# vpc-ccg/tksm

Hardware: AMD Instinct MI355X
Metric: sequenced reads/s (higher is better)
Workload: dtype u8; 1 GPU; Bulk molecules, Badread error+qual model (nanopore2020, identity 84,99,5.5), 24 x 128 Mb random genome, FASTQ; kind=bulk, mean_len=1000, length_distribution=normal(1000, 200), compute_qual=True, contexts_in_flight_per_gpu=3

## Files before the change

__graft_entry__.py:

```python
import os
import subprocess
import sys

ROOT = os.path.dirname(os.path.abspath(__file__))


LLVM_BIN = "/opt/rocm/lib/llvm/bin"
NO_SPILL = ("k_alnf", "k_loop", "k_loopw", "k_err", "k_emit", "k_init")
LOOP_VGPR_LIMIT = 128
NO_SPILL_MDF = ("k_noise_plan", "k_noise_fill", "k_pal_count", "k_pal_write",
                "k_mut_count", "k_mut_write")
NO_SPILL_KDE = ("k_kde_grid", "k_kde_sum", "k_kde_cv_min", "k_kde_cv_sum")
NO_SPILL_ABUND = ("k_abund_compat", "k_abund_hits", "k_abund_msum", "k_abund_mfinish", "k_abund_mtotal", "k_abund_estep")
NO_SPILL_MS = ("k_ms_expand", "k_ms_err_events", "k_ms_qs_events")
NO_SPILL_BM = ("k_bm_match", "k_bm_adapter", "k_bm_exact")
NO_SPILL_MAP = ("k_map_chain", "k_map_sketch", "k_map_seed_write", "k_map_select")
NO_SPILL_MAP_ALIGN = ("k_map_align_path", "k_map_align", "k_map_align_encode")
NO_SPILL_MAP_EXTEND = ("k_map_extend", "k_map_extend_trace")


def kernel_resources(obj):
    import re
    import shutil
    import tempfile
# ... 23 lines not shown
                       ("map_kernels.o", NO_SPILL_MAP), ("map_align_kernels.o", NO_SPILL_MAP_ALIGN),
                       ("map_extend_kernels.o", NO_SPILL_MAP_EXTEND)):
        res = kernel_resources(os.path.join(ROOT, "tksm_amd", "csrc", "_build", obj))
        found = {n: r for n, r in res.items() if any(f"{len(k)}{k}" in n for k in names)}
        missing += [k for k in names if not any(f"{len(k)}{k}" in n for n in found)]
        guarded.update(found)
    if missing:
        raise RuntimeError(f"spill gate: kernels {missing} not found in the code object (renamed?)")
    bad = {n: r for n, r in guarded.items() if r.get("vgpr_spill_count", 0) or r.get("private_segment_fixed_size", 0)}
    if bad:
        raise RuntimeError("spill gate: scratch spills in " + "; ".join(
            f"{n}: {r.get('vgpr_spill_count')} VGPRs spilled, {r.get('private_segment_fixed_size')} B scratch" for n, r in bad.items()))
    return guarded


def build():
    subprocess.check_call(["make", "-s", "-j8", "-C", os.path.join(ROOT, "tksm_amd", "csrc")])
    guarded = check_no_spills()
    loop = [r for n, r in guarded.items() if "6k_loopE" in n]
    if len(loop) != 1 or loop[0]["vgpr_count"] > LOOP_VGPR_LIMIT:
        raise RuntimeError(f"k_loop: {[r['vgpr_count'] for r in loop]} VGPRs, the limit is {LOOP_VGPR_LIMIT}")
    print(f"k_loop: {loop[0]['vgpr_count']} VGPRs (limit {LOOP_VGPR_LIMIT}), no scratch; LDS per wave 256 B x fragment words per lane "
          f"(at most 64: 16 KB) + the 4 KB bounds table of the first thresholds")
    subprocess.check_call(["make", "-s", "-C", os.path.join(ROOT, "oracle")])
    sys.path.insert(0, ROOT)
    import tksm_amd
    from tksm_amd import _lib
    lib = _lib.load()
    missing = [s for s in _lib.SYMBOLS if not hasattr(lib, s)]
    if missing:
        raise RuntimeError(f"libtksmseq.so lacks symbols: {missing}")


def smoke():
    sys.path.insert(0, ROOT)
    sys.path.insert(0, os.path.join(ROOT, "oracle"))
    import numpy as np
    import pyoracle as po
    from tksm_amd.sequence import Sequencer
    models = os.path.join(ROOT, "tksm_amd", "models", "badread")
    err, qs = os.path.join(models, "nanopore2020.error.gz"), os.path.join(models, "nanopore2020.qscore.gz")
    rs = np.random.RandomState(3)
    ref = {f"c{i}": rs.choice(np.frombuffer(b"ACGT", np.uint8), 50_000).tobytes().decode() for i in range(2)}
    s = Sequencer(0)
    for k, v in ref.items():
        s.add_contig(k, v)
# ... 28 lines not shown
```

tksm_amd/csrc/ctx.h:

```cpp
#pragma once
#include <hip/hip_runtime.h>
#include <chrono>

#include <algorithm>
#include <cstdint>
#include <cstdio>
#include <cstdlib>
#include <map>
#include <memory>
#include <mutex>
#include <string>
#include <unordered_map>
#include <vector>

#include "../../include/tksmseq.h"
#include "abund_kernels.h"
#include "host.h"
#include "kernels.h"
#include "tsb_host.h"

using namespace tkh;

#define HIPCHK(ctx, call)                                                                         \
    do {                                                                                          \
// ... 244 lines not shown
    uint64_t total_bases = 0;
    uint32_t pool_blocks = 0;
    std::vector<uint8_t> contig_declared; uint32_t n_declared = 0;
    uint64_t ref_version = 0, wgs_version = ~0ull;
    DevBuf d_wgs_sofar, d_wgs_nameoff, d_wgs_namelen, d_wgs_names;
    DevBuf d_packed, d_blocktab, d_pool, d_contigs, d_stage;
    std::shared_ptr<const tsb::Transcripts> tsb;
    uint64_t tsb_dev_serial = 0, tsb_ref_version = ~0ull;
    DevBuf d_tsb_first, d_tsb_exons, d_tsb_lits, d_tsb_litpool;
    uint64_t tsb_n_lits = 0, tsb_lit_bytes = 0;
    float tsb_plan_ms = 0.f, tsb_write_ms = 0.f;
    uint64_t mut_serial = 0, mut_ref_version = ~0ull;
    DevBuf d_mut_refctg, d_mut_nameoff, d_mut_names, d_mut_delfirst, d_mut_ptfirst, d_mut_delfrom, d_mut_delto, d_mut_ptpos, d_mut_ptinfo, d_mut_insent, d_mut_inspool;

    ErrorModelHost em; QScoreModelHost qm; IdentityHost idm;
    bool em_uniform = false, em_alt0 = false;
    TailModelHost tail; uint64_t tail_version = 0;
    DevBuf d_tail_lx, d_tail_ly, d_tail_cdf, d_tail_chain;
    DevBuf d_pself, d_pseg, d_pt0, d_pt0b, d_cdf32, d_cdf, d_alts, d_altenc, d_nalts, d_qkeys, d_qoff, d_qcnt, d_qcdf, d_qq, d_qtab, d_qent, d_qpairs, d_qguide;

    DevBuf w_rawlen, w_slotcap, w_slotoff, w_outlen, w_ident, w_reclen, w_recoff, w_status, w_scan, w_trace, w_counter,
        w_scratch, w_records, w_istats, w_dstats, w_sums, w_fullpool, w_biglist, w_bigscratch, w_bigtrace;
    unsigned long long full_pool_bytes = 1ull << 30;
    DevBuf f_state, f_frag, f_nb, f_fplanes, f_jmeta[2], f_redo, f_jpopd, f_trace, f_tracefull, f_slow, f_defer, f_defercnt, f_frag2, f_row64;
    std::vector<uint32_t> h_row64;
    DevBuf f_round, f_geoall;
    PinnedBuf h_round, h_geo;
    bool force_slow = false;
    uint32_t tail_cut = 0;
    int tail_wcap = 2048;
    uint32_t tail_wave = 4096;
    uint32_t wave_loop = 16384;
    uint32_t full_rows_cap = 0;
    uint32_t small_aln = 131072;
    uint32_t n_buckets = 16;
    int defer_len = 0;
    int hbm_state_len = 2304;
    std::vector<hipEvent_t> evpool;
    uint32_t last_diag[DIAG_WORDS] = {};
    void* user_out = nullptr; uint64_t user_out_cap = 0;
    bool timing = false;
    int host_threads = 1;
    hipEvent_t ev[6] = {};
    tksmseq_result last{};
    bool have_last = false, have_stats = false;
    DevBuf g_counts, g_nlscan, g_sizes, g_offs, g_plans, g_out;
    tksmseq_gzip_result last_gzip{};
// ... 28 lines not shown
```

tksm_amd/csrc/kernels.h:

```cpp
#pragma once
#include <hip/hip_runtime.h>
#include <stdint.h>

namespace tk {

constexpr uint32_t NO_BLOCK = 0xFFFFFFFFu;
constexpr int BLOCK_SHIFT = 12;
constexpr int WAVES_PER_WG = 4;

struct RefView {
    const uint32_t* packed;
    const uint32_t* blocktab;
    const uint8_t* pool;
    const uint64_t* contigs;
    uint32_t n_contigs;
};

struct BatchView {
    const uint32_t* reads;
    const uint32_t* intervals;
    const uint32_t* mods;
    const uint64_t* literals;
    const uint8_t* litpool;
    const uint32_t* ids;
// ... 110 lines not shown
    CNT_SLOW = 2,
    CNT_FULL_ROWS = 3,
    CNT_EXIT = 4,
    CNT_REDO_JOBS = 8,
    CNT_REDO_WAVES = 9,
    CNT_REDO_LIST = 10,
    CNT_FAIL = 12,
    CNT_FAIL_OR = 13,
    CNT_FAIL_LAST = 14,
    CNT_FAIL_NM = 15,
    CNT_FAIL_REASON = 16,
    CNT_FAIL_QJOB = 24,
    CNT_FAIL_LIST = 25,
    CNT_EARLY_SLOW = 26,
    CNT_EARLY = 27,
    CNT_WORDS = 32
};
enum ExitCause { EXIT_BAND_LOOP = 0, EXIT_SHIFT_LOOP = 1, EXIT_SHIFT_ERR = 2, EXIT_BAND_ERR = 3 };
enum FailBit { FAIL_QUEUE = 0, FAIL_NOROW = 1, FAIL_SHIFT31 = 3, FAIL_SHIFT14 = 4, FAIL_END_CELL = 5, FAIL_WALK = 6 };

struct FastBuffers {
    ReadState* state;
    const uint32_t* row64;
    uint8_t* st_frag;
    uint16_t* st_nb;
    unsigned long long* st_fplanes;
    uint32_t* st_frag2;
    uint32_t* job_meta;
    uint8_t* job_popd;
    void* trace;
    uint32_t* redo_list;
    void* trace_full;
    uint32_t full_rows, full_tg;
    uint32_t full_cl;
    uint32_t* counters;
    uint32_t* job_cnt;
    uint32_t rs, n_ranges;
    const uint32_t* prev_meta; const uint8_t* prev_popd;
    const uint32_t* prefix;
    const uint32_t* base_cur; const uint32_t* base_prev;
    const RangeGeo* geo_cur; const RangeGeo* geo_prev;
    uint32_t* slow_list;
    uint32_t* early_hist;
    uint2* early_list;
    uint32_t* early_slow;
    uint2* defer_list;
    uint32_t* defer_cnt;
// ... 55 lines not shown
```

tksm_amd/csrc/kernels.hip:

```cpp
#include "kernels.h"
#include "loop_filter.h"
#include <type_traits>

namespace tk {

#define DEV __device__ __forceinline__

constexpr int BIG = 1 << 28;
DEV bool is_inf(int v) { return v >= (1 << 27); }

struct Ph4 { uint32_t x, y, z, w; };
enum { ST_ID = 0, ST_PAD = 1, ST_IDENT = 2, ST_DRAW = 3, ST_ALNPOS = 4, ST_QUAL = 5, ST_TAIL = 6 };

DEV Ph4 philox(uint64_t seed, uint64_t read, uint32_t stream, uint32_t n) {
    uint32_t c0 = (uint32_t)read, c1 = (uint32_t)(read >> 32), c2 = stream, c3 = n;
    uint32_t k0 = (uint32_t)seed, k1 = (uint32_t)(seed >> 32);
#pragma unroll
    for (int r = 0; r < 10; r++) {
        const unsigned long long p0 = (unsigned long long)0xD2511F53u * c0, p1 = (unsigned long long)0xCD9E8D57u * c2;
        const uint32_t h0 = (uint32_t)(p0 >> 32), l0 = (uint32_t)p0, h1 = (uint32_t)(p1 >> 32), l1 = (uint32_t)p1;
        uint32_t n0 = h1 ^ c1 ^ k0, n2 = h0 ^ c3 ^ k1;
        c0 = n0; c1 = l1; c2 = n2; c3 = l0;
        k0 += 0x9E3779B9u; k1 += 0xBB67AE85u;
    }
// ... 786 lines not shown
        }
    }
    if (a == 16) {
        uint4 v[4];
#pragma unroll
        for (int q = 0; q < 4; q++) v[q] = c4[4 + q];
#pragma unroll
        for (int q = 0; q < 4; q++) {
            a += !(w < v[q].x) ? 1 : 0; a += !(w < v[q].y) ? 1 : 0; a += !(w < v[q].z) ? 1 : 0; a += !(w < v[q].w) ? 1 : 0;
        }
    }
    return min(a, na);
}

DEV void go_slow(const FastBuffers& FB, uint64_t r, int lane, int cause) {
    if (lane == 0) {
        FB.state[r].slow = 1;
        atomicAdd(&FB.counters[CNT_EXIT + cause], 1u);
        const uint32_t idx = atomicAdd(&FB.counters[CNT_SLOW], 1u);
        FB.slow_list[idx] = (uint32_t)r;
    }
}

DEV uint8_t* frag_row(const FastBuffers& FB, uint64_t r) { return FB.st_frag + (size_t)FB.row64[r] * 64; }
DEV uint16_t* nb_row(const FastBuffers& FB, uint64_t r) { return FB.st_nb + (size_t)FB.row64[r] * 64; }
DEV unsigned long long* planes_row(const FastBuffers& FB, uint64_t r) { return FB.st_fplanes + 2 * ((size_t)FB.row64[r] + 8 * r); }
DEV int planes_words(const FastBuffers& FB, uint64_t r) { return (int)(FB.row64[r + 1] - FB.row64[r]) + 8; }
DEV uint32_t* frag2_row(const FastBuffers& FB, uint64_t r) { return FB.st_frag2 + 4 * ((size_t)FB.row64[r] + r); }
DEV int frag2_words(const FastBuffers& FB, uint64_t r) { return 4 * (int)(FB.row64[r + 1] - FB.row64[r]) + 4; }

DEV uint32_t early_bin(int L, double target) {
    const float sc = (float)L * (float)fmax(0.0, 1.0 - target);
    return (uint32_t)min(255, max(0, (int)(8.0f * __log2f(1.0f + sc))));
}
__global__ __launch_bounds__(256, 7) void k_init(BatchView B, RefView R, ErrModelView EM, IdentView IM, SimParams P,
                                               SimBuffers O, FastBuffers FB) {
#ifndef TKSM_ABLATE
    __builtin_amdgcn_s_setprio(2);
#endif
    const int lane = threadIdx.x & 63, wave = threadIdx.x >> 6, wpw = blockDim.x >> 6;
    const uint64_t r = (uint64_t)blockIdx.x * wpw + wave;
    if (r >= B.n_reads) return;
    uint8_t* frag = lds_raw + (size_t)wave * P.lcap;
    const int k = EM.k;
    const uint64_t g = P.first_read + r * P.stride;
    const int raw_len = (int)O.raw_len[r];
    const int L = raw_len + 2 * k;
    uint32_t status = 0;
    {
        const uint32_t ib = B.reads[2 * r], ic = B.reads[2 * r + 1];
        int o = k;
        for (uint32_t ii = 0; ii < ic; ii++) {
            const Ivl iv = load_interval(B, R, ib + ii);
            const int len = (int)iv.len;
            if (iv.literal) {
                const uint64_t lg = iv.gbase + iv.s;
                for (uint32_t t = (uint32_t)lane; t < (uint32_t)len; t += 64u) {
                    const uint8_t bch = upper(B.litpool[lg + (iv.minus ? (uint32_t)len - 1u - t : t)]);
                    frag[o + t] = iv.minus ? comp(bch) : bch;
                }
            } else
            for (uint32_t t0 = 16u * lane; t0 < (uint32_t)len; t0 += 1024u)
                splice_piece(B, R, iv.gbase + iv.s, (uint32_t)len, false, iv.minus, t0, frag + o + t0);
            wave_sync();
#pragma unroll 1
            for (uint32_t mi = iv.mod_begin; mi < iv.mod_end; mi++) {
// ... 2 lines not shown
                if (lane == 0) frag[o + (iv.minus ? len - 1 - (int)mp : (int)mp)] = iv.minus ? comp((uint8_t)mc) : (uint8_t)mc;
            }
            o += len;
        }
        if (O.tail_len && O.tail_len[r]) tail_fill(O.tail_chain, P.seed, g, frag + o, (int)O.tail_len[r], lane);
    }
    {
        const Ph4 pad = philox(P.seed, g, ST_PAD, 0);
        if (lane < k) {
            frag[lane] = base_char((int)(pad.x >> (2 * lane)));
            frag[k + raw_len + lane] = base_char((int)(pad.y >> (2 * lane)));
        }
    }
    double target;
    if (IM.constant) target = IM.value;
    else {
        const uint32_t u = philox(P.seed, g, ST_IDENT, 0).x;
        const uint32_t idx = u >> 16;
        const double fr = (double)(u & 0xffffu) * (1.0 / 65536.0);
        const double qa = IM.qtab[idx], qb = IM.qtab[idx + 1];
        target = IM.value * (qa + (qb - qa) * fr);
    }
    wave_sync();
    uint8_t* gfrag = frag_row(FB, r);
    unsigned long long* fpl = planes_row(FB, r);
    const int fw_r = planes_words(FB, r), fw2_r = frag2_words(FB, r);
    for (int t = 8 * lane; t < L; t += 512) {
        uint2 c = *reinterpret_cast<const uint2*>(frag + t);
        c.x = ((c.x >> 1) ^ (c.x >> 2)) & 0x03030303u; c.y = ((c.y >> 1) ^ (c.y >> 2)) & 0x03030303u;
        *reinterpret_cast<uint2*>(gfrag + t) = c;
    }
    {
        uint16_t* gnb0 = nb_row(FB, r);
        for (int t = 8 * lane; t < L; t += 512) {
            uint2 c = *reinterpret_cast<const uint2*>(frag + t);
            c.x = ((c.x >> 1) ^ (c.x >> 2)) & 0x03030303u; c.y = ((c.y >> 1) ^ (c.y >> 2)) & 0x03030303u;
            auto two = [](uint32_t b0, uint32_t b1) {
                return (0x1000u | (b0 & 1u) | ((b0 >> 1) << 5)) | ((0x1000u | (b1 & 1u) | ((b1 >> 1) << 5)) << 16);
            };
            uint4 o;
            o.x = two(c.x & 3u, (c.x >> 8) & 3u); o.y = two((c.x >> 16) & 3u, (c.x >> 24) & 3u);
            o.z = two(c.y & 3u, (c.y >> 8) & 3u); o.w = two((c.y >> 16) & 3u, (c.y >> 24) & 3u);
            if (t + 8 > L) {
                const int keep = L - t;
                uint32_t* ow = &o.x;
                for (int x2 = 0; x2 < 8; x2++) if (x2 >= keep) ow[x2 >> 1] &= (x2 & 1) ? 0x0000ffffu : 0xffff0000u;
            }
            *reinterpret_cast<uint4*>(gnb0 + t) = o;
        }
    }
    {
        uint32_t* f2 = frag2_row(FB, r);
        for (int w = lane; w < fw2_r; w += 64) {
            uint32_t word = 0u;
#pragma unroll
            for (int q = 0; q < 4; q++) {
                const int t = 16 * w + 4 * q;
                uint32_t c = t < P.lcap ? *reinterpret_cast<const uint32_t*>(frag + t) : 0u;
                if (t + 4 > L) c = t >= L ? 0u : c & (0xffffffffu >> (8 * (t + 4 - L)));
                const uint32_t codes4 = ((c >> 1) ^ (c >> 2)) & 0x03030303u;
                word |= ((codes4 * 0x40100401u) >> 24) << (24 - 8 * q);
            }
            f2[w] = word;
        }
    }
    bool dirty = false;
    const int nw = (L + 63) >> 6;
    for (int q0 = 0; q0 < fw_r; q0 += 64) {
        unsigned long long mylo = 0ull, myhi = 0ull;
        for (int q = q0; q < min(q0 + 64, nw); q++) {
            const int p = q * 64 + lane;
            const bool valid = p < L;
            const uint8_t c = valid ? frag[p] : (uint8_t)'A';
            const int code = code_of(c);
            dirty |= code < 0;
            const unsigned long long lo = __ballot(valid && (code & 1)), hi = __ballot(valid && (code & 2));
            if (lane == q - q0) { mylo = lo; myhi = hi; }
        }
        if (q0 + lane < fw_r) { ulonglong2 v; v.x = mylo; v.y = myhi; *reinterpret_cast<ulonglong2*>(fpl + 2 * (q0 + lane)) = v; }
    }
    const bool slow = __ballot(dirty) != 0ull;
    if (lane == 0) {
        ReadState S;
        S.errors = 0.0; S.target = target; S.est = 0.0; S.change_count = 0; S.n_base = 0; S.aln_no = 0;
        S.resume_src = -1; S.resume_j = 0; S.stage = 0; S.pending = 0; S.slow = slow ? 1 : 0; S.early = 0;
        S.st_draws = 0; S.st_aligns = 0; S.job = 0; S.raw_len = raw_len; S.res_mt = 0; S.res_cols = 0; S.res_fail = 0; S.pad3 = 0;
        FB.state[r] = S;
        O.status[r] |= status;
        if (slow) { const uint32_t idx = atomicAdd(&FB.counters[CNT_SLOW], 1u); FB.slow_list[idx] = (uint32_t)r; }
        else if (FB.early_hist) atomicAdd(&FB.early_hist[(blockIdx.x & 63u) * 256u + early_bin(L, target)], 1u);
    }
}

DEV void finish_read(const BatchView& B, const SimParams& P, const SimBuffers& O, uint64_t r, int raw_len, int out_len,
                     double identity, uint32_t status, int st_draws, int st_changes, int st_aligns, int L, int st_newlen,
                     int st_strim, int st_etrim, double errors, double target, int lane) {
    if (lane != 0) return;
    if (O.tail_len && !P.quirk_perfect) raw_len -= (int)O.tail_len[r];
    const long long h = pct_hundredths(identity);
    const uint32_t idl = B.ids[2 * r + 1];
    uint64_t rec = 1 + 36 + 8 + ndigits((unsigned)out_len) + 19 + ndigits((unsigned)raw_len) + 15 +
                   ndigits((unsigned long long)(h / 100)) + 3 + 14 + idl + 1;
// ... 43 lines not shown
        for (int jj = 0; jj < 8; jj++) {
            if (jj < k) {
                const uint32_t e = draw_slot(A, jj);
                if ((e >> 15) && (nb[i + jj] & 0x8000u) == 0) r.am |= 1u << jj;
                r.lens |= ((e >> 12) & 7u) << (3 * jj);
            }
        }
    }
    return r;
}

DEV int joined_len(const uint16_t* nb, int p0, int n, int lane) {
    int m = 0;
    for (int q = 0; q < n; q += 64) {
        const int p = q + lane;
        const int len = p < n ? slot_len(nb[p0 + p]) : 0;
        int total;
        (void)prefix_small(len, total);
        m += total;
    }
    return m;
}

DEV void join_out(const uint8_t* frag, const uint16_t* nb, int n, uint8_t* out_seq, int lo, int hi, int lane) {
    int base = 0;
    for (int q = 0; q < n; q += 64) {
        const int p = q + lane;
        uint32_t code = 0; int len = 0; uint8_t orig = 0;
        if (p < n) { code = nb[p]; len = slot_len(code); orig = frag[p]; }
        int total;
        const int off = base + prefix_small(len, total);
        const uint32_t syms = code ? code & 0x3ffu : planar1((uint32_t)orig);
        for (int x2 = 0; x2 < len; x2++) { const int c = off + x2; if (c >= lo && c < hi) out_seq[c - lo] = base_char((int)(((syms >> x2) & 1u) | (((syms >> (5 + x2)) & 1u) << 1))); }
        base += total;
    }
}

#ifndef TKSM_LOOP_N
#define TKSM_LOOP_N 16
#define TKSM_LOOP_K 3
#endif
constexpr int LOOP_N = TKSM_LOOP_N, LOOP_K = TKSM_LOOP_K;
__global__ __launch_bounds__(64) __attribute__((amdgpu_num_vgpr(128))) void k_loop(ErrModelView EM, SimParams P, FastBuffers FB, const uint32_t* __restrict__ order,
                                              uint32_t begin, uint32_t count, int Wl, int from_jobs, uint32_t c0, uint32_t c1) {
#ifndef TKSM_ABLATE
    __builtin_amdgcn_s_setprio(2);
#endif
    uint32_t* lf = reinterpret_cast<uint32_t*>(lds_raw);
    const int lane = threadIdx.x;
    const uint32_t widx = blockIdx.x * 64u + (uint32_t)lane;
    bool act = widx < count;
    uint32_t r = 0, rc = 0;
    if (act) {
        if (!from_jobs) { r = order[begin + widx]; rc = (begin + widx) / FB.rs; }
        else {
// ... 390 lines not shown
                sp->slow = 1;
                atomicAdd(&FB.counters[CNT_EXIT + EXIT_BAND_LOOP], 1u);
                FB.slow_list[atomicAdd(&FB.counters[CNT_SLOW], 1u)] = r;
            }
            return;
        }
        const uint32_t mt = S.res_mt, cols = S.res_cols;
        const double ident = cols ? (double)mt / (double)cols : 0.0;
        if (L <= 1000) errors = (1.0 - ident) * frag_len;
        else {
            const double estimated = (1.0 - ident) * frag_len;
            const double weight = 1000.0 / frag_len;
            errors = estimated * weight + errors * (1.0 - weight);
        }
        aln_no++;
    }
    const uint32_t kmer_range = (uint32_t)(L - k);
    const long long loop_limit = 100ll * L;
    const uint32_t kmask = (1u << (2 * k)) - 1u;
    int cc25 = change_count % 25;
    enum { RUN = 0, NEED_ALN = 1, DONE = 2 };
    int st = RUN;
    int st_aligns = S.st_aligns;
    const uint8_t* gfrag = frag_row(FB, r);
    if (TAIL && L <= 1000) { for (int t = lane; t < L; t += 64) Fw[t] = gfrag[t]; }
    for (;;) {
        while (st == RUN) {
            double est_cur = est_keep;
            if (resume_j == 0) {
                est_cur = 1.0 - div_inrange(errors, frag_len, rcp_len);
                if ((double)change_count > 0.9 * frag_len || est_cur <= target) { st = DONE; st_draws = (int)n; break; }
            }
            const uint32_t nl = n + (uint32_t)lane;
            const bool live = (long long)nl + 1 <= loop_limit;
            const Ph4 d = philox(P.seed, g, ST_DRAW, nl);
            const int di = (int)__umulhi(d.x, kmer_range);
            const int w = di >> 4, o = di & 15;
            const int kidx = (int)((uint32_t)(mk64(f2[w], f2[w + 1]) >> (64 - 2 * o - 2 * k)) & kmask);
            const uint4 seg = EM.pseg[kidx];
            const int na = EM.uniform_nalts ? EM.max_alts : (int)EM.nalts[kidx];
            int cls = EM.type == 0 ? 2 : (d.y < seg.x ? (EM.alt0_noop ? 0 : 3) : 1);
            const int sbase = 8 * ((d.y < seg.y ? 0 : 1) + (d.y < seg.z ? 0 : 1) + (d.y < seg.w ? 0 : 1));
            const uint4* c4 = reinterpret_cast<const uint4*>(EM.cdf32 + (cls == 1 ? (size_t)kidx * 32 + sbase : (size_t)0));
            const uint4 th0 = c4[0], th1 = c4[1];
            size_t at = 0;
            if (cls == 1 || cls == 3) {
                int a = 0;
                if (cls == 1) {
// ... 56 lines not shown
                wave_sync();
                if (stop_at >= 0) {
                    st = NEED_ALN;
                    if (stop_at + 1 < k) { resume_j = stop_at + 1; est_keep = est; n += (uint32_t)src; }
                    else { resume_j = 0; n += (uint32_t)src + 1u; }
                    break;
                }
                resume_j = 0;
                est_cur = 1.0 - div_inrange(errors, frag_len, rcp_len);
                if ((double)change_count > 0.9 * frag_len || est_cur <= target) { st = DONE; st_draws = (int)n + src + 1; break; }
            }
            if (st != RUN) break;
            resume_j = 0;
            if (dead) { st = DONE; st_draws = (int)loop_limit; break; }
            n += 64u;
        }
        if (!TAIL || st != NEED_ALN) break;
        {
            int p0 = 0, nrows = L;
            if (L > 1000) {
                p0 = (int)__umulhi(philox(P.seed, g, ST_ALNPOS, aln_no).x, (uint32_t)(L - 1000 + 1));
                nrows = 1000;
                wave_sync();
                for (int t = lane; t < nrows; t += 64) Fw[t] = gfrag[p0 + t];
            }
            wave_sync();
            const int m = join_window_planar(gnb, p0, nrows, Nw, ownw, wcap, lane);
            wave_sync();
            if (m > wcap) {
                if (early_mode) { to_exact_kernel(); return; }
                break;
            }
            const AlnOut a = band_align<0, false>(Fw, nrows, Nw, ownw, m, lane, nullptr);
            st_aligns++;
            if (is_inf(a.dist)) {
                to_exact_kernel();
                return;
            }
            const int cols = (int)(a.stat & 0xffffu), mt = (int)(a.stat >> 16);
            const double ident = cols ? (double)mt / (double)cols : 0.0;
            if (L <= 1000) errors = (1.0 - ident) * frag_len;
            else {
                const double estimated = (1.0 - ident) * frag_len;
                const double weight = 1000.0 / frag_len;
                errors = estimated * weight + errors * (1.0 - weight);
            }
            aln_no++;
// ... 32 lines not shown
    __builtin_amdgcn_s_setprio(2);
#endif
    const int lane = threadIdx.x & 63, wave = __builtin_amdgcn_readfirstlane(threadIdx.x >> 6), wpw = blockDim.x >> 6;
    const uint32_t widx = blockIdx.x * (uint32_t)wpw + (uint32_t)wave;
    if (widx >= count) return;
    uint64_t r; uint32_t pos;
    if (!from_jobs) { pos = begin + widx; r = (uint64_t)__builtin_amdgcn_readfirstlane((int)order[pos]) & 0xffffffffull; }
    else if (from_jobs == 2) {
        const uint2 e = FB.defer_list[widx];
        r = (uint64_t)__builtin_amdgcn_readfirstlane((int)e.x) & 0xffffffffull;
        pos = (uint32_t)__builtin_amdgcn_readfirstlane((int)e.y) * FB.rs;
    } else {
        const uint32_t target = FB.prefix[c0] + widx;
        uint32_t lo2 = c0, hi2 = c1 - 1;
        while (lo2 < hi2) { const uint32_t mid = (lo2 + hi2 + 1) >> 1; if (FB.prefix[mid] <= target) lo2 = mid; else hi2 = mid - 1; }
        const uint32_t pjob = FB.base_prev[lo2] + (target - FB.prefix[lo2]);
        r = (uint64_t)__builtin_amdgcn_readfirstlane((int)FB.prev_meta[4ull * pjob]) & 0xffffffffull;
        pos = lo2 * FB.rs;
    }
    ReadState S = FB.state[r];
    if (S.stage == 2 || S.slow) return;
    if (S.stage == 0) return;
    uint16_t* gnb = nb_row(FB, r);
    const int per_wave = STATE_IN_HBM ? lds_ncap + 128 : lds_lcap * 3 + lds_ncap + 128;
    uint8_t* lds_wave = lds_raw + (size_t)wave * per_wave;
    uint8_t* frag = STATE_IN_HBM ? frag_row(FB, r) : lds_wave;
    uint16_t* nb = STATE_IN_HBM ? gnb : reinterpret_cast<uint16_t*>(lds_wave + lds_lcap);
    uint8_t* aux = STATE_IN_HBM ? lds_wave : lds_wave + 3 * (size_t)lds_lcap;
    const int k = EM.k;
    const uint64_t g = P.first_read + r * P.stride;
    const int raw_len = __builtin_amdgcn_readfirstlane(S.raw_len);
    const int L = raw_len + 2 * k;
    const uint64_t slot = O.slot_off[r];
    const int cap = __builtin_amdgcn_readfirstlane((int)((O.slot_off[r + 1] - slot) >> 1));
    uint8_t* out_seq = O.scratch + slot;
    uint8_t* out_qual = out_seq + cap;
    if (!STATE_IN_HBM) {
        const uint8_t* gfrag0 = frag_row(FB, r);
        for (int t = lane * 4; t < L; t += 256) *reinterpret_cast<uint32_t*>(frag + t) = *reinterpret_cast<const uint32_t*>(gfrag0 + t);
        for (int t = lane * 2; t < L; t += 128) *reinterpret_cast<uint32_t*>(nb + t) = *reinterpret_cast<const uint32_t*>(gnb + t);
    }
    wave_sync();
    uint32_t status = 0;
    const double frag_len = (double)L;
    const double errors = S.errors;
    const double target = S.target;
    const int change_count = __builtin_amdgcn_readfirstlane(S.change_count), st_draws = __builtin_amdgcn_readfirstlane(S.st_draws);
    int st_aligns = __builtin_amdgcn_readfirstlane(S.st_aligns);
    double identity = 1.0;

    int start_trim, end_trim;
    {
        int v1 = lane < k ? slot_len(nb[lane]) : 0, v2 = lane < k ? slot_len(nb[L - k + lane]) : 0;
        (void)prefix_small(v1, start_trim);
        (void)prefix_small(v2, end_trim);
    }
    const int jcap = min(lds_ncap, cap);
    const int m = joined_len(nb, 0, L, lane);
    int lo = start_trim, hi = end_trim == 0 ? 0 : m - end_trim;
    lo = min(lo, m); hi = max(hi, lo);
    if (m > jcap) { status |= 1; lo = hi = 0; }
    const int out_len = hi - lo;
// ... 82 lines not shown
#ifdef TKSM_ABLATE
            if (P.ablate == 42) { out_qual[i2 - lo] = (uint8_t)(33 + (row & 31)); continue; }
            if (P.ablate == 43 && row >= 0) {
                const uint32_t w = (uint32_t)i2 * 2654435761u;
                const uint32_t a2 = QM.guide[(size_t)row * 64 + (w >> 26)] & 0x7fu;
                out_qual[i2 - lo] = (uint8_t)(33 + QM.pairs[roff + min(a2, rcnt - 1u)].y); continue;
            }
#endif
            if (row >= 0) {
                const uint32_t w = philox(P.seed, g, ST_QUAL, (uint32_t)i2).x;
                uint32_t a2 = QM.guide[(size_t)row * 64 + (w >> 26)];
                if (QM.guide_direct && (a2 & 0x80u)) q = (uint8_t)(a2 & 0x7fu);
                else {
                    uint2 pr = QM.pairs[roff + a2];
                    while (a2 + 1 < rcnt && !(w < pr.x)) { a2++; pr = QM.pairs[roff + a2]; }
                    q = (uint8_t)pr.y;
                }
            }
            out_qual[i2 - lo] = (uint8_t)(q + 33);
        }
    } else {
        identity = 1.0 - errors / frag_len;
    }
    join_out(frag, nb, L, out_seq, lo, hi, lane);
    if (P.quirk_perfect) identity = 1.0;
    finish_read(B, P, O, r, P.quirk_perfect ? out_len : raw_len, out_len, identity, status, st_draws, change_count, st_aligns, L, m,
                start_trim, end_trim, errors, target, lane);
    if (lane == 0) FB.state[r].stage = 2;
}

__global__ void k_collect_unfinished(FastBuffers FB, uint64_t n_reads) {
    const uint64_t r = (uint64_t)blockIdx.x * blockDim.x + threadIdx.x;
    if (r >= n_reads) return;
    ReadState S = FB.state[r];
    if (S.stage != 2 && !S.slow) {
        FB.state[r].slow = 1;
        const uint32_t idx = atomicAdd(&FB.counters[CNT_SLOW], 1u);
        FB.slow_list[idx] = (uint32_t)r;
    }
}

DEV uint32_t range_of_job(const FastBuffers& FB, uint32_t job0) {
    uint32_t rng = 0, hi2 = FB.n_ranges - 1;
    while (rng < hi2) { const uint32_t mid = (rng + hi2 + 1) >> 1; if (FB.base_cur[mid] <= job0) rng = mid; else hi2 = mid - 1; }
    return rng;
}
__global__ __launch_bounds__(64) void k_qjobs(FastBuffers FB, int k, uint32_t count) {
// ... 825 lines not shown
    if (per_cu > 8) per_cu = 8;
    if (per_cu < 1) per_cu = 1;
    return per_cu;
}
hipError_t launch_simulate(const BatchView& b, const RefView& r, const ErrModelView& em, const QsModelView& qm,
                           const IdentView& im, const SimParams& p, const SimBuffers& o, int n_wgs, int wpw, hipStream_t s) {
    if (!b.n_reads) return hipSuccess;
    const int lds = simulate_lds_bytes(p.s_lcap, p.s_ncap, wpw);
    hipError_t e = hipFuncSetAttribute(reinterpret_cast<const void*>(k_simulate<false>), hipFuncAttributeMaxDynamicSharedMemorySize, lds);
    if (e != hipSuccess) return e;
    hipLaunchKernelGGL(k_simulate<false>, dim3(n_wgs), dim3(64 * wpw), lds, s, b, r, em, qm, im, p, o);
    return hipGetLastError();
}
size_t simulate_big_bytes(int lcap, int ncap) { return ((size_t)lcap * 3 + (size_t)ncap * 6 + 255) & ~(size_t)255; }
hipError_t launch_simulate_big(const BatchView& b, const RefView& r, const ErrModelView& em, const QsModelView& qm,
                               const IdentView& im, const SimParams& p, const SimBuffers& o, int n_waves, hipStream_t s) {
    if (!b.n_reads || !n_waves) return hipSuccess;
    hipLaunchKernelGGL(k_simulate<true>, dim3(n_waves), dim3(64), 0, s, b, r, em, qm, im, p, o);
    return hipGetLastError();
}
hipError_t launch_init(const BatchView& b, const RefView& r, const ErrModelView& em, const IdentView& im, const SimParams& p,
                       const SimBuffers& o, const FastBuffers& fb, int wpw, hipStream_t s) {
    if (!b.n_reads) return hipSuccess;
    const int lds = wpw * p.lcap;
    hipError_t e = hipFuncSetAttribute(reinterpret_cast<const void*>(k_init), hipFuncAttributeMaxDynamicSharedMemorySize, lds);
    if (e != hipSuccess) return e;
    hipLaunchKernelGGL(k_init, dim3((unsigned)((b.n_reads + wpw - 1) / wpw)), dim3(64 * wpw), lds, s, b, r, em, im, p, o, fb);
    return hipGetLastError();
}
int err_lds_bytes(int lcap, int ncap, int wpw, bool state_in_hbm) { return wpw * ((state_in_hbm ? 0 : lcap * 3) + ncap + 128); }
hipError_t launch_err(const BatchView& b, const ErrModelView& em, const QsModelView& qm, const SimParams& p, const SimBuffers& o,
                      const FastBuffers& fb, const uint32_t* order, uint32_t begin, uint32_t count, int lds_lcap, int lds_ncap,
                      int from_jobs, uint32_t c0, uint32_t c1, int wpw, bool state_in_hbm, hipStream_t s) {
    if (!count) return hipSuccess;
    const int lds = err_lds_bytes(lds_lcap, lds_ncap, wpw, state_in_hbm);
    auto kern = state_in_hbm ? k_err<true> : k_err<false>;
    hipError_t e = hipFuncSetAttribute(reinterpret_cast<const void*>(kern), hipFuncAttributeMaxDynamicSharedMemorySize, 160 * 1024);
    if (e != hipSuccess) return e;
    hipLaunchKernelGGL(kern, dim3((count + wpw - 1) / wpw), dim3(64 * wpw), lds, s, b, em, qm, p, o, fb, order, begin, count, lds_lcap,
                       lds_ncap, from_jobs, c0, c1);
    return hipGetLastError();
}
constexpr int LOOP_WL_MAX = 64;
int loop_lds_words(int lcap) {
    static const int wl_max = [] { const char* e = getenv("TKSMSEQ_LOOP_WL"); return e ? std::max(4, atoi(e) & ~3) : LOOP_WL_MAX; }();
    return std::min(wl_max, (((lcap + 15) / 16 + 1) + 3) & ~3);
}
hipError_t launch_loop(const ErrModelView& em, const SimParams& p, const FastBuffers& fb, const uint32_t* order, uint32_t begin,
                       uint32_t count, int lcap, int from_jobs, uint32_t c0, uint32_t c1, hipStream_t s) {
    if (!count) return hipSuccess;
    const int Wl = loop_lds_words(lcap);
    hipLaunchKernelGGL(k_loop, dim3((count + 63) / 64), dim3(64), (size_t)Wl * 256 + tklf::LOOP_FILTER_BYTES, s, em, p, fb, order, begin, count, Wl, from_jobs, c0, c1);
    return hipGetLastError();
// ... 161 lines not shown
```

tksm_amd/csrc/run.cpp:

```cpp
#include "../../include/tksmseq.h"

#include <hip/hip_runtime.h>

#include <algorithm>
#include <cstdio>
#include <cstring>
#include <cstdlib>
#include <string>

#include "ctx.h"

#define TRY(call) do { const int rc_ = (call); if (rc_ != TKSMSEQ_OK) return rc_; } while (0)

static tk::BatchView batch_view(const tksmseq_batch* b) {
    return tk::BatchView{b->reads.as<uint32_t>(), b->intervals.as<uint32_t>(), b->mods.as<uint32_t>(), b->literals.as<uint64_t>(),
                         b->litpool.as<uint8_t>(), b->ids.as<uint32_t>(), b->idpool.as<uint8_t>(), b->n_reads, (uint32_t)b->n_literals};
}
static tk::RefView ref_view(const tksmseq_ctx* ctx) {
    return tk::RefView{ctx->d_packed.as<uint32_t>(), ctx->d_blocktab.as<uint32_t>(), ctx->d_pool.as<uint8_t>(),
                       ctx->d_contigs.as<uint64_t>(), (uint32_t)ctx->contig_names.size()};
}

static int apply_tail(tksmseq_ctx* ctx, tksmseq_batch* b, const tksmseq_run_params* p) {
    const bool want = p->mode == TKSMSEQ_MODE_BADREAD && ctx->tail.enabled && b->n_reads > 0;
// ... 174 lines not shown
        for (uint32_t c = 0; c < FB.n_ranges; c++) {
            r_ncap[c] = (uint32_t)pl.capf(b->raw_len[b->order[last_pos(c)]]);
            r_tg[c] = ((r_ncap[c] + 31) & ~31u) / 16 + 1;
            tot_trace += (uint64_t)FB.rs * r_tg[c]; tot_popd += (uint64_t)FB.rs * r_ncap[c];
        }
        ctx->h_row64.resize(n + 1);
        for (uint64_t r = 0; r < n; r++) { ctx->h_row64[r] = (uint32_t)nblk; nblk += ((uint64_t)b->raw_len[r] + 2 * pl.k + 63) / 64 + 1; }
        ctx->h_row64[n] = (uint32_t)nblk;
        nrb = (size_t)FB.n_ranges * 128;
        round_bytes = 2 * nrb + 1024;
        geo_off = (((size_t)(FB.n_ranges + 1) * 12 + 63) & ~(size_t)63);
        geo_bytes = geo_off + (size_t)FB.n_ranges * 2 * sizeof(tk::RangeGeo);
        FB.full_cl = ((((uint32_t)pl.ncap + 31) & ~31u) / 4 + 16 + 3) & ~3u;
        FB.full_tg = FB.full_cl + (FB.full_cl / 4 + 3) / 4 + 1;
        FB.full_rows = (uint32_t)std::max<uint64_t>(64, std::min<uint64_t>(jcap, (4ull << 30) / ((uint64_t)FB.full_tg * 64)) & ~63ull);
        full_rows_fit = FB.full_rows;
        if (ctx->full_rows_cap) FB.full_rows = std::min(FB.full_rows, std::max(64u, ctx->full_rows_cap & ~63u));
        early_on = ctx->early_tail > 0 && ctx->tail_cut == 0 && ctx->tail_wave > 0 && tk::tail_lds_bytes(pl.lcap) <= 65536 && n >= 16ull * ctx->early_tail;
    }
    int grow_buffers() {
        if (nblk >= (1ull << 32)) { ctx->err = "batch too large (split it)"; return TKSMSEQ_ELIMIT; }
        HIPCHK(ctx, ctx->f_state.ensure(n * sizeof(tk::ReadState) + 64));
        HIPCHK(ctx, ctx->f_row64.ensure((n + 1) * 4 + 64));
        HIPCHK(ctx, ctx->f_frag.ensure(nblk * 64 + 256));
        HIPCHK(ctx, ctx->f_nb.ensure(nblk * 128 + 256));
        HIPCHK(ctx, ctx->f_fplanes.ensure((nblk + 8 * n) * 16 + 256));
        HIPCHK(ctx, ctx->f_frag2.ensure((4 * nblk + 4 * n) * 4 + 1024));
        for (DevBuf& m : ctx->f_jmeta) HIPCHK(ctx, m.ensure(jcap * 16 + 64));
        HIPCHK(ctx, ctx->f_jpopd.ensure(tot_popd + 64));
        HIPCHK(ctx, ctx->f_round.ensure(round_bytes + 64));
        HIPCHK(ctx, ctx->f_geoall.ensure(geo_bytes + 64));
        HIPCHK(ctx, ctx->f_trace.ensure(tot_trace * 64 + 64));
        HIPCHK(ctx, ctx->f_redo.ensure(jcap * 4 + 64));
        HIPCHK(ctx, ctx->f_tracefull.ensure((size_t)FB.full_rows * FB.full_tg * 64 + 64));
        HIPCHK(ctx, ctx->f_slow.ensure(n * 4 + 64));
        HIPCHK(ctx, ctx->f_defer.ensure(n * 8 + 64));
        HIPCHK(ctx, ctx->f_defercnt.ensure((size_t)FB.n_ranges * 128 + 64));
        HIPCHK(ctx, ctx->h_round.ensure(round_bytes));
        HIPCHK(ctx, ctx->h_geo.ensure(geo_bytes));
        HIPCHK(ctx, hipMemcpyAsync(ctx->f_row64.p, ctx->h_row64.data(), (n + 1) * 4, hipMemcpyHostToDevice, s));
        FB.state = ctx->f_state.as<tk::ReadState>(); FB.st_frag = ctx->f_frag.as<uint8_t>(); FB.st_nb = ctx->f_nb.as<uint16_t>();
        FB.st_fplanes = ctx->f_fplanes.as<unsigned long long>(); FB.st_frag2 = ctx->f_frag2.as<uint32_t>(); FB.row64 = ctx->f_row64.as<uint32_t>();
        FB.trace = ctx->f_trace.p;
        FB.redo_list = ctx->f_redo.as<uint32_t>();
        FB.trace_full = ctx->f_tracefull.p; FB.counters = reinterpret_cast<uint32_t*>(ctx->f_round.as<uint8_t>() + nrb);
        FB.slow_list = ctx->f_slow.as<uint32_t>();
        FB.early_hist = nullptr; FB.early_list = nullptr; FB.early_slow = nullptr;
        if (early_on) {
            HIPCHK(ctx, ctx->f_early.ensure(65536 + (size_t)EARLY_CAP * 12 + 64));
            FB.early_hist = ctx->f_early.as<uint32_t>();
            FB.early_list = reinterpret_cast<uint2*>(ctx->f_early.as<uint8_t>() + 65536);
            FB.early_slow = reinterpret_cast<uint32_t*>(ctx->f_early.as<uint8_t>() + 65536 + (size_t)EARLY_CAP * 8);
            HIPCHK(ctx, hipMemsetAsync(ctx->f_early.p, 0, 65536, s));
        }
        FB.defer_list = ctx->f_defer.as<uint2>(); FB.defer_cnt = ctx->f_defercnt.as<uint32_t>(); FB.defer_len = ctx->defer_len;
        HIPCHK(ctx, hipMemsetAsync(ctx->f_defercnt.p, 0, (size_t)FB.n_ranges * 128, s));
        FB.prefix = ctx->f_geoall.as<uint32_t>(); FB.base_prev = FB.prefix + (FB.n_ranges + 1); FB.base_cur = FB.prefix + 2 * (FB.n_ranges + 1);
        FB.geo_cur = reinterpret_cast<tk::RangeGeo*>(ctx->f_geoall.as<uint8_t>() + geo_off); FB.geo_prev = FB.geo_cur + FB.n_ranges;
        return TKSMSEQ_OK;
    }
    void select_set(uint32_t round) {
        const int z = round & 1, y = z ^ 1;
        FB.job_meta = ctx->f_jmeta[z].as<uint32_t>(); FB.prev_meta = ctx->f_jmeta[y].as<uint32_t>();
        FB.prev_popd = FB.job_popd = ctx->f_jpopd.as<uint8_t>();
// ... 35 lines not shown
            Bucket bk;
            bk.begin = (uint32_t)i0; bk.count = (uint32_t)(i1 - i0);
            bk.lcap = (int)((mx + 2 * pl.k + 7) & ~7u); bk.ncap = (int)pl.capf(mx);
            bk.hbm = bk.lcap > ctx->hbm_state_len;
            bk.wpw = tk::WAVES_PER_WG;
            while (bk.wpw > 1 && tk::err_lds_bytes(bk.lcap, bk.ncap, bk.wpw, bk.hbm) > 64 * 1024) bk.wpw >>= 1;
            buckets.push_back(bk);
            i0 = i1;
        }
    }
    int prepare() {
        size_ranges();
        TRY(grow_buffers());
        select_set(0);
        HIPCHK(ctx, hipStreamSynchronize(s));
        memset(ctx->h_geo.p, 0, geo_bytes);
        const size_t nr1 = FB.n_ranges + 1;
        hprefix = ctx->h_geo.as<uint32_t>(); hbase_prev = hprefix + nr1; hbase_cur = hprefix + 2 * nr1;
        hrg = reinterpret_cast<tk::RangeGeo*>(ctx->h_geo.as<uint8_t>() + geo_off);
        for (uint32_t c = 0; c <= FB.n_ranges; c++) hbase_cur[c] = hbase_prev[c] = c * FB.rs;
        HIPCHK(ctx, place_ranges());
        cnt = ctx->h_round.as<uint32_t>() + nrb / 4;
        make_buckets();
        HIPCHK(ctx, hipMemsetAsync(ctx->f_nb.p, 0, nblk * 128, s));
        HIPCHK(ctx, hipMemsetAsync(ctx->f_round.p, 0, round_bytes, s));
        TRY(tick(GAP));
        pl.mark("buffers ready");
        return TKSMSEQ_OK;
    }
    int launch_side(uint32_t upto) {
        if (upto <= n_side || side_launches + 2 >= 1024) return TKSMSEQ_OK;
        const int k2 = (int)(side_launches % tksmseq_ctx::N_SIDE);
        HelperStream& h = ctx->side[k2];
        tk::SimBuffers O2 = pl.O;
        O2.read_list = ctx->f_slow.as<uint32_t>() + n_side; O2.n_work = upto - n_side;
        O2.work_counter = ctx->w_counter.as<unsigned long long>() + 1 + side_launches;
        O2.trace = pl.O.trace + ((size_t)pl.n_wgs * pl.wpw + (size_t)k2 * tksmseq_ctx::SIDE_WAVES) * pl.trace_words;
        HIPCHK(ctx, h.fork_from(s));
        const uint64_t want = (O2.n_work + pl.wpw - 1) / pl.wpw;
        const int wgs = (int)std::max<uint64_t>(1, std::min<uint64_t>(want, (uint64_t)(tksmseq_ctx::SIDE_WAVES / pl.wpw)));
        HIPCHK(ctx, tk::launch_simulate(pl.B, pl.R, pl.EM, pl.QM, pl.IM, pl.P, O2, wgs, pl.wpw, h.stream));
        HIPCHK(ctx, h.launched());
        n_side = upto; side_launches++;
        return TKSMSEQ_OK;
    }
    int launch_early(const std::vector<uint32_t>& copies) {
        uint32_t hist[256] = {};
// ... 325 lines not shown
```

Before: 15.39 million reads/s.

## Drop the byte fragment buffer and derive codes from packed planes

Removes the per-read byte-per-base fragment array from HBM. k_init now writes the 2-bit packed words, the nb slots and the bit planes in a single fused pass over LDS, with tail masking applied inline, so the separate memset of the nb buffer is no longer needed. The alignment window in k_loop rebuilds its codes from the frag2 words, and k_err reconstructs output bases from the nb slot codes alone, which frees one lcap of LDS per wave. The intent is less HBM traffic and memory footprint plus more LDS headroom, at the cost of extra unpacking arithmetic and a dependence on nb being fully initialised for every position.

```diff
diff --git a/__graft_entry__.py b/__graft_entry__.py
--- a/__graft_entry__.py
+++ b/__graft_entry__.py
@@ -69,6 +69,8 @@
         raise RuntimeError(f"k_loop: {[r['vgpr_count'] for r in loop]} VGPRs, the limit is {LOOP_VGPR_LIMIT}")
     print(f"k_loop: {loop[0]['vgpr_count']} VGPRs (limit {LOOP_VGPR_LIMIT}), no scratch; LDS per wave 256 B x fragment words per lane "
           f"(at most 64: 16 KB) + the 4 KB bounds table of the first thresholds")
+    for kern, tag in (("k_init", "6k_initE"), ("k_err<false>", "5k_errILb0EE"), ("k_err<true>", "5k_errILb1EE")):
+        print(f"{kern}: " + ", ".join(f"{r['vgpr_count']} VGPRs, no scratch" for n, r in guarded.items() if tag in n))
     subprocess.check_call(["make", "-s", "-C", os.path.join(ROOT, "oracle")])
     sys.path.insert(0, ROOT)
     import tksm_amd
diff --git a/tksm_amd/csrc/ctx.h b/tksm_amd/csrc/ctx.h
--- a/tksm_amd/csrc/ctx.h
+++ b/tksm_amd/csrc/ctx.h
@@ -290,7 +290,7 @@
     DevBuf w_rawlen, w_slotcap, w_slotoff, w_outlen, w_ident, w_reclen, w_recoff, w_status, w_scan, w_trace, w_counter,
         w_scratch, w_records, w_istats, w_dstats, w_sums, w_fullpool, w_biglist, w_bigscratch, w_bigtrace;
     unsigned long long full_pool_bytes = 1ull << 30;
-    DevBuf f_state, f_frag, f_nb, f_fplanes, f_jmeta[2], f_redo, f_jpopd, f_trace, f_tracefull, f_slow, f_defer, f_defercnt, f_frag2, f_row64;
+    DevBuf f_state, f_nb, f_fplanes, f_jmeta[2], f_redo, f_jpopd, f_trace, f_tracefull, f_slow, f_defer, f_defercnt, f_frag2, f_row64;
     std::vector<uint32_t> h_row64;
     DevBuf f_round, f_geoall;
     PinnedBuf h_round, h_geo;
diff --git a/tksm_amd/csrc/kernels.h b/tksm_amd/csrc/kernels.h
--- a/tksm_amd/csrc/kernels.h
+++ b/tksm_amd/csrc/kernels.h
@@ -156,7 +156,6 @@
 struct FastBuffers {
     ReadState* state;
     const uint32_t* row64;
-    uint8_t* st_frag;
     uint16_t* st_nb;
     unsigned long long* st_fplanes;
     uint32_t* st_frag2;
diff --git a/tksm_amd/csrc/kernels.hip b/tksm_amd/csrc/kernels.hip
--- a/tksm_amd/csrc/kernels.hip
+++ b/tksm_amd/csrc/kernels.hip
@@ -832,7 +832,6 @@
     }
 }
 
-DEV uint8_t* frag_row(const FastBuffers& FB, uint64_t r) { return FB.st_frag + (size_t)FB.row64[r] * 64; }
 DEV uint16_t* nb_row(const FastBuffers& FB, uint64_t r) { return FB.st_nb + (size_t)FB.row64[r] * 64; }
 DEV unsigned long long* planes_row(const FastBuffers& FB, uint64_t r) { return FB.st_fplanes + 2 * ((size_t)FB.row64[r] + 8 * r); }
 DEV int planes_words(const FastBuffers& FB, uint64_t r) { return (int)(FB.row64[r + 1] - FB.row64[r]) + 8; }
@@ -843,6 +842,7 @@
     const float sc = (float)L * (float)fmax(0.0, 1.0 - target);
     return (uint32_t)min(255, max(0, (int)(8.0f * __log2f(1.0f + sc))));
 }
+__host__ __device__ inline int init_lds_stride(int lcap) { return (lcap + 15) & ~15; }
 __global__ __launch_bounds__(256, 7) void k_init(BatchView B, RefView R, ErrModelView EM, IdentView IM, SimParams P,
                                                SimBuffers O, FastBuffers FB) {
 #ifndef TKSM_ABLATE
@@ -851,7 +851,7 @@
     const int lane = threadIdx.x & 63, wave = threadIdx.x >> 6, wpw = blockDim.x >> 6;
     const uint64_t r = (uint64_t)blockIdx.x * wpw + wave;
     if (r >= B.n_reads) return;
-    uint8_t* frag = lds_raw + (size_t)wave * P.lcap;
+    uint8_t* frag = lds_raw + (size_t)wave * init_lds_stride(P.lcap);
     const int k = EM.k;
     const uint64_t g = P.first_read + r * P.stride;
     const int raw_len = (int)O.raw_len[r];
@@ -900,62 +900,48 @@
         target = IM.value * (qa + (qb - qa) * fr);
     }
     wave_sync();
-    uint8_t* gfrag = frag_row(FB, r);
     unsigned long long* fpl = planes_row(FB, r);
-    const int fw_r = planes_words(FB, r), fw2_r = frag2_words(FB, r);
-    for (int t = 8 * lane; t < L; t += 512) {
-        uint2 c = *reinterpret_cast<const uint2*>(frag + t);
-        c.x = ((c.x >> 1) ^ (c.x >> 2)) & 0x03030303u; c.y = ((c.y >> 1) ^ (c.y >> 2)) & 0x03030303u;
-        *reinterpret_cast<uint2*>(gfrag + t) = c;
-    }
-    {
-        uint16_t* gnb0 = nb_row(FB, r);
-        for (int t = 8 * lane; t < L; t += 512) {
-            uint2 c = *reinterpret_cast<const uint2*>(frag + t);
-            c.x = ((c.x >> 1) ^ (c.x >> 2)) & 0x03030303u; c.y = ((c.y >> 1) ^ (c.y >> 2)) & 0x03030303u;
-            auto two = [](uint32_t b0, uint32_t b1) {
-                return (0x1000u | (b0 & 1u) | ((b0 >> 1) << 5)) | ((0x1000u | (b1 & 1u) | ((b1 >> 1) << 5)) << 16);
-            };
-            uint4 o;
-            o.x = two(c.x & 3u, (c.x >> 8) & 3u); o.y = two((c.x >> 16) & 3u, (c.x >> 24) & 3u);
-            o.z = two(c.y & 3u, (c.y >> 8) & 3u); o.w = two((c.y >> 16) & 3u, (c.y >> 24) & 3u);
-            if (t + 8 > L) {
-                const int keep = L - t;
-                uint32_t* ow = &o.x;
-                for (int x2 = 0; x2 < 8; x2++) if (x2 >= keep) ow[x2 >> 1] &= (x2 & 1) ? 0x0000ffffu : 0xffff0000u;
-            }
-            *reinterpret_cast<uint4*>(gnb0 + t) = o;
-        }
-    }
-    {
-        uint32_t* f2 = frag2_row(FB, r);
-        for (int w = lane; w < fw2_r; w += 64) {
-            uint32_t word = 0u;
-#pragma unroll
-            for (int q = 0; q < 4; q++) {
-                const int t = 16 * w + 4 * q;
-                uint32_t c = t < P.lcap ? *reinterpret_cast<const uint32_t*>(frag + t) : 0u;
-                if (t + 4 > L) c = t >= L ? 0u : c & (0xffffffffu >> (8 * (t + 4 - L)));
-                const uint32_t codes4 = ((c >> 1) ^ (c >> 2)) & 0x03030303u;
-                word |= ((codes4 * 0x40100401u) >> 24) << (24 - 8 * q);
-            }
-            f2[w] = word;
-        }
-    }
+    uint16_t* gnb0 = nb_row(FB, r);
+    uint32_t* f2 = frag2_row(FB, r);
+    const int nb64 = (int)(FB.row64[r + 1] - FB.row64[r]);
+    const int fw_r = nb64 + 8, fw2_r = 4 * nb64 + 4;
     bool dirty = false;
-    const int nw = (L + 63) >> 6;
-    for (int q0 = 0; q0 < fw_r; q0 += 64) {
-        unsigned long long mylo = 0ull, myhi = 0ull;
-        for (int q = q0; q < min(q0 + 64, nw); q++) {
-            const int p = q * 64 + lane;
-            const bool valid = p < L;
-            const uint8_t c = valid ? frag[p] : (uint8_t)'A';
-            const int code = code_of(c);
-            dirty |= code < 0;
-            const unsigned long long lo = __ballot(valid && (code & 1)), hi = __ballot(valid && (code & 2));
-            if (lane == q - q0) { mylo = lo; myhi = hi; }
-        }
-        if (q0 + lane < fw_r) { ulonglong2 v; v.x = mylo; v.y = myhi; *reinterpret_cast<ulonglong2*>(fpl + 2 * (q0 + lane)) = v; }
+    for (int w0 = 0; w0 < 4 * fw_r; w0 += 64) {
+        const int w = w0 + lane, t = 16 * w, nv = L - t;
+        uint4 c = make_uint4(0u, 0u, 0u, 0u);
+        if (nv > 0) c = *reinterpret_cast<const uint4*>(frag + t);
+        const uint32_t c4[4] = {c.x, c.y, c.z, c.w};
+        uint32_t word = 0u, lo16 = 0u, hi16 = 0u, sc[8];
+#pragma unroll
+        for (int q = 0; q < 4; q++) {
+            const int nq = nv - 4 * q;
+            const uint32_t vm = nq >= 4 ? 0xffffffffu : nq <= 0 ? 0u : (1u << (8 * nq)) - 1u;
+            const uint32_t cd = ((c4[q] >> 1) ^ (c4[q] >> 2)) & 0x03030303u & vm;
+            const uint32_t b0 = cd & 0x01010101u, b1 = (cd >> 1) & 0x01010101u;
+            dirty |= ((c4[q] ^ (0x41414141u + 2u * b0 + 6u * b1 + 11u * (b0 & b1))) & vm) != 0u;
+            word |= ((cd * 0x40100401u) >> 24) << (24 - 8 * q);
+            lo16 |= ((b0 * 0x01020408u) >> 24) << (4 * q);
+            hi16 |= ((b1 * 0x01020408u) >> 24) << (4 * q);
+            const uint32_t cv = cd | (vm & 0x04040404u);
+            const uint32_t y0 = __builtin_amdgcn_perm(cv, cv, 0x0c010c00u), y1 = __builtin_amdgcn_perm(cv, cv, 0x0c030c02u);
+            sc[2 * q] = (y0 & 0x00010001u) | ((y0 & 0x00020002u) << 4) | ((y0 & 0x00040004u) << 10);
+            sc[2 * q + 1] = (y1 & 0x00010001u) | ((y1 & 0x00020002u) << 4) | ((y1 & 0x00040004u) << 10);
+        }
+        if (w < fw2_r) f2[w] = word;
+        if (w < 4 * nb64) {
+            uint4* d = reinterpret_cast<uint4*>(gnb0 + t);
+            d[0] = make_uint4(sc[0], sc[1], sc[2], sc[3]);
+            d[1] = make_uint4(sc[4], sc[5], sc[6], sc[7]);
+        }
+        const int pc = (int)(lo16 | (hi16 << 16));
+        const uint32_t p0 = (uint32_t)dpp_mov<0x00, 0xf>(0, pc), p1 = (uint32_t)dpp_mov<0x55, 0xf>(0, pc),
+                       p2 = (uint32_t)dpp_mov<0xaa, 0xf>(0, pc), p3 = (uint32_t)dpp_mov<0xff, 0xf>(0, pc);
+        if ((lane & 3) == 0 && (w >> 2) < fw_r) {
+            ulonglong2 v;
+            v.x = mk64((p2 & 0xffffu) | (p3 << 16), (p0 & 0xffffu) | (p1 << 16));
+            v.y = mk64((p2 >> 16) | (p3 & 0xffff0000u), (p0 >> 16) | (p1 & 0xffff0000u));
+            *reinterpret_cast<ulonglong2*>(fpl + 2 * (w >> 2)) = v;
+        }
     }
     const bool slow = __ballot(dirty) != 0ull;
     if (lane == 0) {
@@ -1045,15 +1031,15 @@
     return m;
 }
 
-DEV void join_out(const uint8_t* frag, const uint16_t* nb, int n, uint8_t* out_seq, int lo, int hi, int lane) {
+DEV void join_out(const uint16_t* nb, int n, uint8_t* out_seq, int lo, int hi, int lane) {
     int base = 0;
     for (int q = 0; q < n; q += 64) {
         const int p = q + lane;
-        uint32_t code = 0; int len = 0; uint8_t orig = 0;
-        if (p < n) { code = nb[p]; len = slot_len(code); orig = frag[p]; }
+        uint32_t code = 0; int len = 0;
+        if (p < n) { code = nb[p]; len = slot_len(code); }
         int total;
         const int off = base + prefix_small(len, total);
-        const uint32_t syms = code ? code & 0x3ffu : planar1((uint32_t)orig);
+        const uint32_t syms = code & 0x3ffu;
         for (int x2 = 0; x2 < len; x2++) { const int c = off + x2; if (c >= lo && c < hi) out_seq[c - lo] = base_char((int)(((syms >> x2) & 1u) | (((syms >> (5 + x2)) & 1u) << 1))); }
         base += total;
     }
@@ -1490,8 +1476,17 @@
     enum { RUN = 0, NEED_ALN = 1, DONE = 2 };
     int st = RUN;
     int st_aligns = S.st_aligns;
-    const uint8_t* gfrag = frag_row(FB, r);
-    if (TAIL && L <= 1000) { for (int t = lane; t < L; t += 64) Fw[t] = gfrag[t]; }
+    auto window_codes = [&](int p0, int nrows) {
+        for (int t = 16 * lane; t < nrows; t += 1024) {
+            const int x = p0 + t, w = x >> 4, o = x & 15;
+            const uint32_t c16 = (uint32_t)((mk64(f2[w], f2[w + 1]) << (2 * o)) >> 32);
+            uint32_t b[4] = {0u, 0u, 0u, 0u};
+#pragma unroll
+            for (int j = 0; j < 16; j++) b[j >> 2] |= ((c16 >> (30 - 2 * j)) & 3u) << (8 * (j & 3));
+            *reinterpret_cast<uint4*>(Fw + t) = make_uint4(b[0], b[1], b[2], b[3]);
+        }
+    };
+    if (TAIL && L <= 1000) window_codes(0, L);
     for (;;) {
         while (st == RUN) {
             double est_cur = est_keep;
@@ -1594,7 +1589,7 @@
                 p0 = (int)__umulhi(philox(P.seed, g, ST_ALNPOS, aln_no).x, (uint32_t)(L - 1000 + 1));
                 nrows = 1000;
                 wave_sync();
-                for (int t = lane; t < nrows; t += 64) Fw[t] = gfrag[p0 + t];
+                window_codes(p0, nrows);
             }
             wave_sync();
             const int m = join_window_planar(gnb, p0, nrows, Nw, ownw, wcap, lane);
@@ -1673,11 +1668,10 @@
     if (S.stage == 2 || S.slow) return;
     if (S.stage == 0) return;
     uint16_t* gnb = nb_row(FB, r);
-    const int per_wave = STATE_IN_HBM ? lds_ncap + 128 : lds_lcap * 3 + lds_ncap + 128;
+    const int per_wave = STATE_IN_HBM ? lds_ncap + 128 : lds_lcap * 2 + lds_ncap + 128;
     uint8_t* lds_wave = lds_raw + (size_t)wave * per_wave;
-    uint8_t* frag = STATE_IN_HBM ? frag_row(FB, r) : lds_wave;
-    uint16_t* nb = STATE_IN_HBM ? gnb : reinterpret_cast<uint16_t*>(lds_wave + lds_lcap);
-    uint8_t* aux = STATE_IN_HBM ? lds_wave : lds_wave + 3 * (size_t)lds_lcap;
+    uint16_t* nb = STATE_IN_HBM ? gnb : reinterpret_cast<uint16_t*>(lds_wave);
+    uint8_t* aux = STATE_IN_HBM ? lds_wave : lds_wave + 2 * (size_t)lds_lcap;
     const int k = EM.k;
     const uint64_t g = P.first_read + r * P.stride;
     const int raw_len = __builtin_amdgcn_readfirstlane(S.raw_len);
@@ -1687,8 +1681,6 @@
     uint8_t* out_seq = O.scratch + slot;
     uint8_t* out_qual = out_seq + cap;
     if (!STATE_IN_HBM) {
-        const uint8_t* gfrag0 = frag_row(FB, r);
-        for (int t = lane * 4; t < L; t += 256) *reinterpret_cast<uint32_t*>(frag + t) = *reinterpret_cast<const uint32_t*>(gfrag0 + t);
         for (int t = lane * 2; t < L; t += 128) *reinterpret_cast<uint32_t*>(nb + t) = *reinterpret_cast<const uint32_t*>(gnb + t);
     }
     wave_sync();
@@ -1817,7 +1809,7 @@
     } else {
         identity = 1.0 - errors / frag_len;
     }
-    join_out(frag, nb, L, out_seq, lo, hi, lane);
+    join_out(nb, L, out_seq, lo, hi, lane);
     if (P.quirk_perfect) identity = 1.0;
     finish_read(B, P, O, r, P.quirk_perfect ? out_len : raw_len, out_len, identity, status, st_draws, change_count, st_aligns, L, m,
                 start_trim, end_trim, errors, target, lane);
@@ -2689,13 +2681,13 @@
 hipError_t launch_init(const BatchView& b, const RefView& r, const ErrModelView& em, const IdentView& im, const SimParams& p,
                        const SimBuffers& o, const FastBuffers& fb, int wpw, hipStream_t s) {
     if (!b.n_reads) return hipSuccess;
-    const int lds = wpw * p.lcap;
+    const int lds = wpw * init_lds_stride(p.lcap);
     hipError_t e = hipFuncSetAttribute(reinterpret_cast<const void*>(k_init), hipFuncAttributeMaxDynamicSharedMemorySize, lds);
     if (e != hipSuccess) return e;
     hipLaunchKernelGGL(k_init, dim3((unsigned)((b.n_reads + wpw - 1) / wpw)), dim3(64 * wpw), lds, s, b, r, em, im, p, o, fb);
     return hipGetLastError();
 }
-int err_lds_bytes(int lcap, int ncap, int wpw, bool state_in_hbm) { return wpw * ((state_in_hbm ? 0 : lcap * 3) + ncap + 128); }
+int err_lds_bytes(int lcap, int ncap, int wpw, bool state_in_hbm) { return wpw * ((state_in_hbm ? 0 : lcap * 2) + ncap + 128); }
 hipError_t launch_err(const BatchView& b, const ErrModelView& em, const QsModelView& qm, const SimParams& p, const SimBuffers& o,
                       const FastBuffers& fb, const uint32_t* order, uint32_t begin, uint32_t count, int lds_lcap, int lds_ncap,
                       int from_jobs, uint32_t c0, uint32_t c1, int wpw, bool state_in_hbm, hipStream_t s) {
diff --git a/tksm_amd/csrc/run.cpp b/tksm_amd/csrc/run.cpp
--- a/tksm_amd/csrc/run.cpp
+++ b/tksm_amd/csrc/run.cpp
@@ -220,7 +220,6 @@
         if (nblk >= (1ull << 32)) { ctx->err = "batch too large (split it)"; return TKSMSEQ_ELIMIT; }
         HIPCHK(ctx, ctx->f_state.ensure(n * sizeof(tk::ReadState) + 64));
         HIPCHK(ctx, ctx->f_row64.ensure((n + 1) * 4 + 64));
-        HIPCHK(ctx, ctx->f_frag.ensure(nblk * 64 + 256));
         HIPCHK(ctx, ctx->f_nb.ensure(nblk * 128 + 256));
         HIPCHK(ctx, ctx->f_fplanes.ensure((nblk + 8 * n) * 16 + 256));
         HIPCHK(ctx, ctx->f_frag2.ensure((4 * nblk + 4 * n) * 4 + 1024));
@@ -237,7 +236,7 @@
         HIPCHK(ctx, ctx->h_round.ensure(round_bytes));
         HIPCHK(ctx, ctx->h_geo.ensure(geo_bytes));
         HIPCHK(ctx, hipMemcpyAsync(ctx->f_row64.p, ctx->h_row64.data(), (n + 1) * 4, hipMemcpyHostToDevice, s));
-        FB.state = ctx->f_state.as<tk::ReadState>(); FB.st_frag = ctx->f_frag.as<uint8_t>(); FB.st_nb = ctx->f_nb.as<uint16_t>();
+        FB.state = ctx->f_state.as<tk::ReadState>(); FB.st_nb = ctx->f_nb.as<uint16_t>();
         FB.st_fplanes = ctx->f_fplanes.as<unsigned long long>(); FB.st_frag2 = ctx->f_frag2.as<uint32_t>(); FB.row64 = ctx->f_row64.as<uint32_t>();
         FB.trace = ctx->f_trace.p;
         FB.redo_list = ctx->f_redo.as<uint32_t>();
@@ -319,7 +318,6 @@
         HIPCHK(ctx, place_ranges());
         cnt = ctx->h_round.as<uint32_t>() + nrb / 4;
         make_buckets();
-        HIPCHK(ctx, hipMemsetAsync(ctx->f_nb.p, 0, nblk * 128, s));
         HIPCHK(ctx, hipMemsetAsync(ctx->f_round.p, 0, round_bytes, s));
         TRY(tick(GAP));
         pl.mark("buffers ready");
```

Result: faster. 16.13 million reads/s (median of 6 runs) (+4.8%).
